# hartikainen/mujoco_mpc

Hardware: AMD Instinct MI355X
Metric: candidate rollouts/s (horizon x samples) (higher is better)
Workload: dtype f64

## Files before the change

mujoco_mpc_amd/csrc/core.h:

```cpp
#pragma once
#include "dmath.h"
#include "model.h"
#include "linalg.h"
#include "philox.h"

#ifdef MJPC_EMU
static thread_local double *g_emu_lds = nullptr;
static thread_local int g_emu_r = 0;
typedef const KParams *KP;
DEV const KParams *kp_generic(KP k) { return k; }
DEV double *lds_base() { return g_emu_lds; }
DEV int cand_index() { return g_emu_r; }
DEV int uniform_i(int v) { return v; }
#else
extern __shared__ __align__(16) double g_lds[];
typedef const __attribute__((address_space(4))) KParams *KP;
DEV const KParams *kp_generic(KP k) {
  unsigned long long v = (unsigned long long)k;
  unsigned lo = __builtin_amdgcn_readfirstlane((unsigned)v), hi = __builtin_amdgcn_readfirstlane((unsigned)(v >> 32));
  KP u = (KP)(((unsigned long long)hi << 32) | lo);
  return (const KParams *)u;
}
DEV double *lds_base() { return g_lds; }
DEV int cand_index() { return (int)blockIdx.x; }
// ... 292 lines not shown
  c.nsingle = nsingle;
  make_contact_rows(c, n_nc); PROF(c, 5);
  make_impedance(c, 0, c.nefc, 1); PROF(c, 7);
#endif
  ctx_close(c);
}
#if MJPC_HELPER
DEV_NOINLINE void ph_noncontact(KP Kc, int t) {
  Ctx c; ctx_open(c, Kc, 1);
  int nsingle, n_nc;
#if MJPC_SIDE_COM
  if (c.M->neq_connect) { if (!flag_wait(c.misc + HX_COM, t + 1)) c.warning |= WARN_SYNC; }
#endif
  make_noncontact_rows(c, &nsingle, &n_nc);
  if (LANE == 0) { c.misc[HX_NC_NSINGLE] = nsingle; c.misc[HX_NC_ROWS] = n_nc; }
  flag_set(c.misc + HX_NCROWS, t + 1);
  PROFW(c, 1);
  make_impedance(c, 0, n_nc, 0);
  PROFW(c, 4);
  if (!flag_wait(c.misc + HX_SWEEP, t + 1)) c.warning |= WARN_SYNC;
  subtree_sums(c, 1);
  flag_set(c.misc + HX_SUBSUM, t + 1);
  PROFW(c, 5);
  ctx_close(c);
}
#endif
template <int NVT>
DEV_NOINLINE void ph_smooth(KP Kc, int t) {
  Ctx c; ctx_open(c, Kc, 1);
#if MJPC_HELPER
#if MJPC_SIDE_COM
  kinematics_rest(c);
  com_pos(c);
  flag_set(c.misc + HX_COM, t + 1);
#endif
  velocity_stage<NVT>(c, Kc, t + 1);
#else
  crb_and_factor<NVT>(c); PROF(c, 3);
  velocity_stage<NVT>(c, Kc, 0); PROF(c, 6);
#endif
  ctx_close(c);
}
#if MJPC_HELPER
template <int NVT>
DEV_NOINLINE void ph_inertia(KP Kc, int t) {
  Ctx c; ctx_open(c, Kc, 1);
#if MJPC_SIDE_COM
  if (!flag_wait(c.misc + HX_COM, t + 1)) c.warning |= WARN_SYNC;
#endif
  crb_and_factor<NVT>(c);
  flag_set(c.misc + HX_MFACT, t + 1);
  ctx_close(c);
}
#endif
template <int NVT>
DEV_NOINLINE void ph_solve(KP Kc, int last, int t) {
  Ctx c; ctx_open(c, Kc);
  c.hseq = t * 256;
  solve_constraints<NVT>(c); PROF(c, 8);
#if MJPC_HELPER
  if (NVT > 0) { if (c.M->cone == 1) flag_set(c.misc + HX_JOBW, JOBW(++c.hseq, 0, 0)); }
  else {
    if (LANE == 0) c.misc[HX_UNREAD_KIND] = 0;
    flag_set(c.misc + HX_UNREAD_SEQ, ++c.hseq);
  }
#endif
  if (!last && !(c.warning & (WARN_CONTACTFULL | WARN_CNSTRFULL)) && bad_values(c.qacc, c.M->nv)) c.warning |= WARN_BADQACC;
  ctx_close(c);
}
template <int NVT>
DEV_NOINLINE void ph_noslip(KP Kc, int last) {
  Ctx c; ctx_open(c, Kc);
  if (!(c.warning & (WARN_CONTACTFULL | WARN_CNSTRFULL | WARN_SYNC | WARN_BADQACC))) {
    noslip_pass<NVT>(c);
    if (!last && bad_values(c.qacc, c.M->nv)) c.warning |= WARN_BADQACC;
  }
  ctx_close(c);
}
#if MJPC_HELPER
template <int NVT>
DEV_NOINLINE void ph_solve_helper(KP Kc, int t) {
  Ctx c; ctx_open(c, Kc, 1);
  int k = WAVE_ID() - 1;
  static_for<0, MJPC_NH>([&](auto Kc_) { constexpr int KK = decltype(Kc_)::value; if (k == KK) solver_helper_loop<NVT, KK>(c, t * 256); });
}
#endif

struct CostOut { double cost; int warning; };
DEV_NOINLINE CostOut ph_residual_cost(KP Kc, int t, int last) {
  Ctx c; ctx_open(c, Kc, 1);
  const KParams *K = c.K;
  const DevModel &M = *c.M;
  const DevTask &T = M.task;
  Rows R = out_rows(K);
  if (last) PFOR(k, M.nu) R.actions[t * M.nu + k] = (K->H > 1) ? c.ctrl[k] : 0.0;
  if (t == 0 && cand_index() == 0 && K->frame) {
    int nb = M.nbody, ns = M.nsite;
    double *f = K->frame;
    PFOR(i, 3 * nb) { f[i] = c.xpos[i]; f[12 * nb + 3 * ns + i] = c.subtree_com[i]; f[15 * nb + 3 * ns + i] = c.subtree_linvel[i]; }
    PFOR(i, 9 * nb) f[3 * nb + i] = c.xmat[i];
    PFOR(i, 3 * ns) f[12 * nb + i] = c.site_xpos[i];
  }
  task_residual(c, c.residual); PROF(c, 9); PROFW(c, 9);
  PFOR(i, R.nr) R.residual[t * R.nr + i] = c.residual[i];
  PFOR(i, T.num_trace) {
    int id = MI(task.trace_objid)[i], ty = MI(task.trace_objtype)[i];
    const double *src = ty == 6 ? c.site_xpos + 3 * id : (ty == 5 ? c.geom_xpos + 3 * id : (ty == 1 ? c.xipos + 3 * id : c.xpos + 3 * id));
    d_copy3(R.trace + t * R.ntr + 3 * i, src);
  }
  CostOut o;
  o.cost = cost_value(c, c.residual);
  if (LANE == 0) R.costs[t] = o.cost;
  o.warning = c.warning;
  PROF(c, 10); PROFW(c, 10);
  ctx_close(c);
  return o;
}

template <int NVT>
DEV void prefactor_body(Ctx &c) {
  const DevModel &M = *c.M;
  {
    int nv = M.nv, nvp = M.nvp;
    double h = M.timestep;
    PFOR(e, nv * nvp) { int i = e / nvp, j = e - i * nvp; c.qL[e] = c.qM[e] + ((i == j) ? h * MD(dof_damping)[i] : 0.0); }
    if (M.nidrv) {
      SYNC();
      if (LANE == 0)
        for (int k = 0; k < M.nidrv; k++) {
          int i = MI(idrv_e)[3 * k], j = MI(idrv_e)[3 * k + 1], a = MI(idrv_e)[3 * k + 2];
          if (a >= 0 && MI(actuator_forcelimited)[a]) {
            double f = c.actuator_force[a];
            if (f <= MD(actuator_forcerange)[2 * a] || f >= MD(actuator_forcerange)[2 * a + 1]) continue;
          }
          double v = h * MD(idrv_c)[k];
          c.qL[i * nvp + j] += v;
          if (i != j) c.qL[j * nvp + i] += v;
        }
      SYNC();
    }
    chol_factor<NVT>(c.qL, c.Linv, c.scr_a, nv, nvp, c.M->tree_ok);
  }
}
template <int NVT>
DEV_NOINLINE void ph_prefactor(KP Kc) {
  Ctx c; ctx_open(c, Kc, 1);
  const DevModel &M = *c.M;
  if (M.any_damping && !M.int_dense && M.noslip_iterations <= 0) prefactor_body<NVT>(c);
  PROFW(c, 11);
  ctx_close(c);
}

DEV void implicit_rne_columns(Ctx &c, double *A, double h) {
  const DevModel &M = *c.M;
  const int nv = M.nv, nvp = M.nvp, nb = M.nbody;
  double *S = lay_ptr(c.K, lds_base(), c.K->L.efc_J);
  int B = M.int_scratch / (18 * nb);
  B = B > NLANE ? NLANE : B;
#define S_(b, k) S[((b) * 18 + (k)) * B + LANE]
  for (int j0 = 0; j0 < nv; j0 += B) {
    const int j = j0 + LANE;
    if (LANE < B && j < nv) {
      for (int pass = 0; pass < 2; pass++) {
        const double sgn = pass ? -1.0 : 1.0;
        for (int b = 1; b < nb; b++) {
          const int p = MIH(body_parentid)[b];
          double cv[6], ca[6];
// ... 286 lines not shown
```

mujoco_mpc_amd/csrc/solver.h:

```cpp
#pragma once
#include "linalg.h"

#ifdef MJPC_EMU
#define LS_RPL 192
#define LS_CPL 64
#else
#define LS_RPL 3
#define LS_CPL 1
#endif

template <int DIMT, bool WRITE = true>
DEV double constraint_update(Ctx &c, int hess, const double *jar) {
  double cost = 0;
  const int nefc = c.nefc, ncon = c.ncon, nv = c.M->nv, nvp = c.M->nvp, stride = c.M->con_stride;
  const int nslot = (nefc + NLANE - 1) / NLANE, ncslot = (ncon + NLANE - 1) / NLANE;
  int rtype[LS_RPL], rdof[LS_RPL];
  double rD[LS_RPL], rx[LS_RPL], rfl[LS_RPL], rR[LS_RPL], rJ[LS_RPL];
  int cdim[LS_CPL], crow[LS_CPL], ctype[LS_CPL];
  double cmu[LS_CPL], cfr[LS_CPL][DIMT], cX[LS_CPL][DIMT], cD[LS_CPL][DIMT];
#pragma unroll
  for (int k = 0; k < LS_RPL; k++) {
    if (k >= nslot) break;
    int i = LANE + NLANE * k, ic = i < nefc ? i : nefc - 1;
    rtype[k] = c.efc_type[ic]; rD[k] = c.efc_D[ic]; rx[k] = jar[ic]; rfl[k] = c.efc_floss[ic]; rR[k] = c.efc_R[ic];
// ... 285 lines not shown
        else {
          i = (int)((sqrtf(8.0f * (float)e + 1.0f) - 1.0f) * 0.5f);
          while ((i + 1) * (i + 2) / 2 <= e) i++;
          while (i * (i + 1) / 2 > e) i--;
          j = e - i * (i + 1) / 2;
        }
      }
      ii[g] = i; jj[g] = j;
    }
    double hp[G], hq[G], hn[G];
#pragma unroll
    for (int g = 0; g < G; g++) { hp[g] = 0; hq[g] = 0; hn[g] = 0; }
    for (int a = 0; a < npos8; a += 8) {
      double x[G][8], y[G][8];
#pragma unroll
      for (int g = 0; g < G; g++)
#pragma unroll
        for (int k = 0; k < 8; k++) { x[g][k] = JH[(a + k) * nvp + ii[g]]; y[g][k] = JH[(a + k) * nvp + jj[g]]; }
#pragma unroll
      for (int g = 0; g < G; g++)
#pragma unroll
        for (int k = 0; k < 8; k += 2) { hp[g] += x[g][k] * y[g][k]; hq[g] += x[g][k + 1] * y[g][k + 1]; }
    }
    for (int a = npos8; a < ntot; a += 4) {
      double x[G][4], y[G][4];
#pragma unroll
      for (int g = 0; g < G; g++)
#pragma unroll
        for (int k = 0; k < 4; k++) { x[g][k] = JH[(a + k) * nvp + ii[g]]; y[g][k] = JH[(a + k) * nvp + jj[g]]; }
#pragma unroll
      for (int g = 0; g < G; g++)
#pragma unroll
        for (int k = 0; k < 4; k++) hn[g] += x[g][k] * y[g][k];
    }
#pragma unroll
    for (int g = 0; g < G; g++) {
      int e = e0 + g * stride, i = ii[g], j = jj[g];
      if (e >= nent) continue;
      double h = hp[g] + hq[g];
      if (j == nv) {
        double gr = c.Ma[i] - c.qfrc_smooth[i] - (c.sgl[i] + c.sgl[2 * nv + i]) - h;
        c.grad[i] = gr;
        c.Mgrad[i] = gr;
      } else {
        h = c.qM[i * nvp + j] + (h - hn[g]);
        if (i == j) h += c.sgl[nv + i] + c.sgl[3 * nv + i];
        c.qH[i * nvp + j] = h;
      }
    }
  }
}

DEV void newton_gradient(Ctx &c, int grad_only) {
  const DevModel &M = *c.M;
  const int nvp = M.nvp;
  PROF(c, 13);
  int npos, nneg;
  newton_lists(c, &npos, &nneg);
  PROF(c, 15);
  newton_fill(c, npos, nneg);
  PROF(c, 19);
  SYNC();
  newton_entries(c, npos, nneg, grad_only);
  if (c.cross) { if (LANE == 0) c.misc[MISC_QH_DENSE] = 1; }
  else {
    PFOR(e, M.nzpair) c.qH[MI(zpair_i)[e] * nvp + MI(zpair_j)[e]] = 0;
    if (LANE == 0) c.misc[MISC_QH_DENSE] = 0;
  }
  SYNC();
  PROF(c, 16);
}

template <int NVT>
DEV double cost_at_smooth(Ctx &c) {
  double *jar = c.efc_pos;
  mat_rows_times<NVT>(c, c.qacc_smooth, c.scr_b, jar);
  PFOR(r, c.nefc) jar[r] -= c.efc_aref[r];
  SYNC();
  double part = c.M->maxdim <= 3 ? constraint_update<3, false>(c, 0, jar) : constraint_update<6, false>(c, 0, jar);
  return 0.0 + wave_sum(part);
}

#if MJPC_HELPER
template <int NVT> DEV void worker_loop(Ctx &c, int W, int last);
template <int NVT> DEV void ls_records_build(Ctx &c);
template <int NVT, int K>
DEV void solver_helper_loop(Ctx &c, int seq) {
  if (K == MJPC_NH - 1 && c.nefc > 0) {
    double cs = cost_at_smooth<NVT>(c);
    if (LANE == 0) c.red[2] = cs;
    const int mute_csm = c.K->fault == 1 && cand_index() == 1 && seq == 2 * 256;
    if (!mute_csm) flag_set(c.misc + HX_CSM, seq / 256 + 1);
  }
  if constexpr (NVT > 0) {
    if (K == 0 && c.nefc > 0) { ls_records_build<NVT>(c); flag_set(c.misc + HX_LSREC, seq / 256 + 1); }
    worker_loop<NVT>(c, K, seq);
  }
}
#endif
template <int NVT>
DEV void newton_direction(Ctx &c) {
  const int nv = NVT > 0 ? NVT : c.M->nv, nvp = NVT > 0 ? NVP_OF(NVT) : c.M->nvp;
  chol_factor_solve<NVT>(c.qH, c.Hinv, c.vtmp, c.Mgrad, nv, nvp, c.M->tree_ok && !c.cross);
  PROF(c, 17);
}
#ifndef MJPC_EMU
template <int NVT>
DEV void newton_direction_sum(Ctx &c, const LDLExtra &ex) {
  chol_factor_solve_reg<NVT>(c.qH, c.Mgrad, NVP_OF(NVT), c.M->tree_ok && !c.cross, &ex);
  PROF(c, 17);
}
#endif

struct LSPoint { double cost, d1, d2; };
template <int DIMT>
struct LSData {
  double lo[LS_RPL], hi[LS_RPL], hD[LS_RPL], F[LS_RPL], X[LS_RPL], V[LS_RPL], DV[LS_RPL], DVV[LS_RPL];
  double U0[LS_CPL][DIMT], UV[LS_CPL][DIMT], E[LS_CPL][DIMT], mu[LS_CPL], Dm[LS_CPL], VV[LS_CPL];
  int on[LS_CPL];
  int nslot, ncslot;
};

template <int DIMT>
DEV void ls_load(Ctx &c, LSData<DIMT> &d) {
  const int nefc = c.nefc, ncon = c.ncon, last = c.nefc - 1;
  d.nslot = (nefc + NLANE - 1) / NLANE; d.ncslot = (ncon + NLANE - 1) / NLANE;
#pragma unroll
  for (int k = 0; k < LS_RPL; k++) {
    d.lo[k] = -1; d.hi[k] = 1; d.hD[k] = 0; d.F[k] = 0; d.X[k] = 0; d.V[k] = 0; d.DV[k] = 0; d.DVV[k] = 0;
    if (k < d.nslot) {
      int r = LANE + NLANE * k, rc = r < nefc ? r : last;
      int type = c.efc_type[rc];
      double D = c.efc_D[rc], v = c.efc_jv[rc], x = c.efc_jar[rc], f = c.efc_floss[rc], Rf = c.efc_R[rc] * f;
      int quad = r < nefc && type != CNSTR_CONTACT_ELLIPTIC;
      int fric = quad && type <= CNSTR_FRICTION_TENDON;
      D = quad ? D : 0.0; v = quad ? v : 0.0;
      d.X[k] = quad ? x : 0.0; d.V[k] = v; d.hD[k] = 0.5 * D; d.DV[k] = D * v; d.DVV[k] = D * v * v;
      d.lo[k] = fric ? -Rf : (quad ? -1e300 : -1.0); d.hi[k] = fric ? Rf : (quad ? 0.0 : 1.0); d.F[k] = fric ? f : 0.0;
    }
  }
#pragma unroll
  for (int q = 0; q < LS_CPL; q++) {
    d.on[q] = 0; d.mu[q] = 0; d.Dm[q] = 0; d.VV[q] = 0;
#pragma unroll
    for (int j = 0; j < DIMT; j++) { d.U0[q][j] = 0; d.UV[q][j] = 0; d.E[q][j] = 0; }
    if (q < d.ncslot) {
      int ci = LANE + NLANE * q, cic = ci < ncon ? ci : ncon - 1;
      int dim = c.con_i[cic * CONI_STRIDE];
      int i = c.con_i[cic * CONI_STRIDE + 3];
      const double *cc = c.contact + cic * c.M->con_stride;
      int type = c.efc_type[i];
      double mu = cc[CON_MU], fr[DIMT], Dj[DIMT], jv[DIMT], jr[DIMT];
#pragma unroll
      for (int j = 0; j < DIMT; j++) {
        int rj = i + j < nefc ? i + j : last;
        fr[j] = j == 0 ? mu : cc[CON_FRICTION + j - 1];
        Dj[j] = c.efc_D[rj]; jv[j] = c.efc_jv[rj]; jr[j] = c.efc_jar[rj];
      }
      int on = ci < ncon && dim > 1 && type == CNSTR_CONTACT_ELLIPTIC;
      d.on[q] = on; d.mu[q] = on ? mu : 0.0;
      d.Dm[q] = on ? Dj[0] * fast_rcp(mu * mu * (1 + mu * mu)) : 0.0;
      double vv = 0;
#pragma unroll
      for (int j = 0; j < DIMT; j++) {
        int use = on && j < dim;
        double uv = jv[j] * fr[j];
        d.U0[q][j] = use ? jr[j] * fr[j] : 0.0; d.UV[q][j] = use ? uv : 0.0;
        d.E[q][j] = use ? Dj[j] * fast_rcp(fr[j] * fr[j]) : 0.0;
        if (j > 0) vv += use ? uv * uv : 0.0;
      }
      d.VV[q] = vv;
    }
  }
}

template <int DIMT>
DEV LSPoint ls_eval(const LSData<DIMT> &d, double q0, double q1, double q2, double a) {
  LSPoint p; p.cost = 0; p.d1 = 0; p.d2 = 0;
#pragma unroll
// ... 165 lines not shown
```

mujoco_mpc_amd/csrc/solver_reg.h:

```cpp
#pragma once
#ifndef MJPC_EMU

template <int NVT> struct HLay {
  static constexpr int G0 = 64 / NVT;
  static constexpr int G = G0 < 1 ? 1 : (G0 > NVT ? NVT : G0);
  static constexpr int CB = (NVT + G - 1) / G;
};
DEV int readlane_i(int v, int lane) { return __builtin_amdgcn_readlane(v, lane); }
#define LSR_STRIDE 7
#define LSC_STRIDE 17
#define LS_ROWREC(c) ((c).efc_JA + 64)
#define LS_CONREC(c) ((c).efc_JA + 64 + (c).M->nefcmax * LSR_STRIDE)

template <int NVT>
DEV void hblock_add_rows(const Ctx &c, double *h, unsigned long long mask, int rbase, double wlane, int hi, int j0) {
  constexpr int nvp = NVP_OF(NVT), CB = HLay<NVT>::CB;
  while (mask) {
    int b0 = (int)__builtin_ctzll(mask); mask &= mask - 1;
    int b1 = b0; double sel1 = 0.0;
    if (mask) { b1 = (int)__builtin_ctzll(mask); mask &= mask - 1; sel1 = 1.0; }
    double w0 = readlane_d(wlane, b0), w1 = readlane_d(wlane, b1) * sel1;
    const double *r0p = c.efc_J + (rbase + b0) * nvp, *r1p = c.efc_J + (rbase + b1) * nvp;
    double x0 = r0p[hi], x1 = r1p[hi];
    double y0[CB], y1[CB];
#pragma unroll
    for (int q = 0; q < CB; q++) { y0[q] = r0p[j0 + q]; y1[q] = r1p[j0 + q]; }
    __builtin_amdgcn_sched_barrier(0);
#ifdef MJPC_LEAN_LDS
    if constexpr (HLay<NVT>::G == 1) {
      double s0 = w0 * x0, s1 = w1 * x1;
#pragma unroll
      for (int q = 0; q < CB; q++) {
        const bool up = j0 + q > hi;
        h[q] = __builtin_fma(up ? w0 * y0[q] : s0, up ? x0 : y0[q], h[q]);
        h[q] = __builtin_fma(up ? w1 * y1[q] : s1, up ? x1 : y1[q], h[q]);
      }
    } else
#endif
    {
      double s0 = w0 * x0, s1 = w1 * x1;
#pragma unroll
      for (int q = 0; q < CB; q++) { h[q] = __builtin_fma(s0, y0[q], h[q]); h[q] = __builtin_fma(s1, y1[q], h[q]); }
    }
  }
}

template <int NVT>
DEV void hblock_init(const Ctx &c, double *hq, int hi, int j0) {
  constexpr int nvp = NVP_OF(NVT), CB = HLay<NVT>::CB;
#pragma unroll
  for (int q = 0; q < CB; q++) hq[q] = c.qM[hi * nvp + j0 + q];
  const int nefc = c.nefc, ns = c.nsingle;
  for (int base = 0; base < nefc; base += NLANE) {
    int r = base + LANE, rc = r < nefc ? r : nefc - 1;
    int st = c.efc_state[rc], type = c.efc_type[rc];
    double D = c.efc_D[rc];
    int flag = r < nefc && r >= ns && st == STATE_QUADRATIC;
    (void)type;
    unsigned long long mask = __builtin_amdgcn_ballot_w64(flag != 0);
    hblock_add_rows<NVT>(c, hq, mask, base, D, hi, j0);
  }
}

template <int NVT>
DEV void newton_grad_reg(Ctx &c, int hi, int hg, bool hact) {
  constexpr int nvp = NVP_OF(NVT), G = HLay<NVT>::G;
  const int ns = c.nsingle, n = c.nefc - ns;
  double part = 0;
  const int trips = (n + G - 1) / G;
  for (int t0 = 0; t0 < trips; t0 += 8) {
    double f[8], j[8];
#pragma unroll
    for (int u = 0; u < 8; u++) {
      int rr = (t0 + u) * G + hg;
      int r = ns + (rr < n ? rr : 0);
      f[u] = c.efc_force[r]; j[u] = c.efc_J[r * nvp + hi];
    }
    __builtin_amdgcn_sched_barrier(0);
#pragma unroll
    for (int u = 0; u < 8; u++) { int rr = (t0 + u) * G + hg; double pr = j[u] * f[u]; part += (rr < n) ? pr : 0.0; }
    __builtin_amdgcn_sched_barrier(0);
  }
  double *sc = c.efc_JA;
  if (hact) sc[hg * NVT + hi] = part;
  SYNC();
  if (LANE < NVT) {
    int i = LANE;
    double jtf = 0;
#pragma unroll
    for (int g = 0; g < G; g++) jtf += sc[g * NVT + i];
    double gr = c.Ma[i] - c.qfrc_smooth[i] - (c.sgl[i] + c.sgl[2 * NVT + i]) - jtf;
    c.grad[i] = gr;
    c.Mgrad[i] = gr;
  }
  SYNC();
}

#define JOBW(seq, np, kind) (((seq) << 4) | ((np) << 2) | (kind))
static_assert(HX_WDONE + MJPC_NH <= HX_WDONE_END, "one done slot per worker");
#define CONE_BASE(c) ((c).efc_JA + 64 + (c).M->nefcmax * LSR_STRIDE + (c).M->nconmax * LSC_STRIDE)
#define CONE_DOFS(c) ((unsigned char *)CONE_BASE(c))
#define CONE_ITEMS(c) ((unsigned short *)(CONE_BASE(c) + ((c).M->nconmax * NVT + 7) / 8))
#define CONE_PARTIAL(c, w) (CONE_BASE(c) + ((c).M->nconmax * NVT + 7) / 8 + ((c).M->nconmax * NVT + 3) / 4 + (w) * (NVT * NVP_OF(NVT)))

template <int NVT, int DIMT>
DEV void cone_rows(const Ctx &c, double *part, int p0, int pstep) {
  constexpr int nvp = NVP_OF(NVT);
  const int nitems = uniform_i(c.misc[HX_NITEMS]), stride = c.M->con_stride;
  const unsigned short *items = CONE_ITEMS(c);
  const double *crec = LS_CONREC(c);
  for (int it0 = p0 * NLANE; it0 < nitems; it0 += pstep * NLANE) {
    const int it = it0 + LANE;
    const bool valid = it < nitems;
    const int item = items[valid ? it : 0];
    const int ci = item & 255, a = item >> 8;
    const int info = ((const int *)(crec + ci * LSC_STRIDE + 14))[0];
    const int r0 = info >> 16, dim = (info >> 8) & 255;
    const unsigned char *dofs = CONE_DOFS(c) + ci * NVT;
    const int i = dofs[a];
    const int st = c.efc_state[r0];
    const double *cf = c.contact + ci * stride + CON_H;
    double P[DIMT], Q[DIMT], T[DIMT], ji[DIMT];
#pragma unroll
    for (int k = 0; k < DIMT; k++) { P[k] = cf[k]; Q[k] = cf[6 + k]; T[k] = cf[12 + k]; }
    const double *Jr = c.efc_J + r0 * nvp;
#pragma unroll
    for (int k = 0; k < DIMT; k++) ji[k] = Jr[(DIMT <= 3 || k < dim ? k : 0) * nvp + i];
    __builtin_amdgcn_sched_barrier(0);
    const bool active = valid && st == STATE_CONE;
#if defined(MJPC_PROFILE) && !defined(MJPC_EMU)
    if (MJPC_PROFILE_WAVE != 0 && WAVE_ID() == MJPC_PROFILE_WAVE) { int na_ = __builtin_popcountll(__builtin_amdgcn_ballot_w64(active)); if (LANE == 0) { c.prof[23] += na_; c.prof[22] += (it0 == p0 * NLANE); } }
#endif
    if constexpr (DIMT > 3) {
#pragma unroll
      for (int k = 3; k < DIMT; k++) { const bool in = k < dim; P[k] = in ? P[k] : 0.0; Q[k] = in ? Q[k] : 0.0; T[k] = in ? T[k] : 0.0; ji[k] = in ? ji[k] : 0.0; }
    }
    double pi = P[0] * ji[0], qi = Q[1] * ji[1];
#pragma unroll
    for (int k = 1; k < DIMT; k++) { pi += P[k] * ji[k]; if (k > 1) qi += Q[k] * ji[k]; }
    double t[DIMT];
    t[0] = P[0] * pi + Q[0] * ji[0];
#pragma unroll
    for (int k = 1; k < DIMT; k++) t[k] = P[k] * pi - Q[k] * qi + (T[k] * T[k]) * ji[k];
    double *prow = part + i * nvp;
    PROFW(c, 16);
    for (int b = 0; __builtin_amdgcn_ballot_w64(active && b <= a) != 0; b += 2) {
      const bool on0 = active && b <= a, on1 = active && b + 1 <= a;
      const int j0 = dofs[on0 ? b : 0], j1 = dofs[on1 ? b + 1 : 0];
      double x0[DIMT], x1[DIMT];
#pragma unroll
      for (int k = 0; k < DIMT; k++) { x0[k] = Jr[(DIMT <= 3 || k < dim ? k : 0) * nvp + j0]; x1[k] = Jr[(DIMT <= 3 || k < dim ? k : 0) * nvp + j1]; }
      __builtin_amdgcn_sched_barrier(0);
      double v0 = t[0] * x0[0], v1 = t[0] * x1[0];
#pragma unroll
      for (int k = 1; k < DIMT; k++) { v0 += t[k] * x0[k]; v1 += t[k] * x1[k]; }
      if (on0) __builtin_amdgcn_ds_atomic_fadd_f64((__attribute__((address_space(3))) double *)(prow + j0), v0);
      if (on1) __builtin_amdgcn_ds_atomic_fadd_f64((__attribute__((address_space(3))) double *)(prow + j1), v1);
    }
  }
}

DEV int jobw_load(const Ctx &c) { return __builtin_amdgcn_readfirstlane(__hip_atomic_load(c.misc + HX_JOBW, __ATOMIC_RELAXED, __HIP_MEMORY_SCOPE_WORKGROUP)); }
DEV int job_post(Ctx &c, int kind, int &side_in) {
  if (c.M->cone != 1) return 0;
  const int seq = ++c.hseq;
  const int np = MJPC_NH + (side_in ? 1 : 0);
  flag_set(c.misc + HX_JOBW, JOBW(seq, np, kind));
  return np;
}
DEV void job_wait(Ctx &c, int np) {
  const int seq = c.hseq;
  for (int k = 0; k < np; k++) if (!flag_wait(c.misc + HX_WDONE + k, seq)) c.warning |= WARN_SYNC;
}
template <int NVT, int DIMT>
DEV void worker_job(Ctx &c, int W, int np, int seq) {
  constexpr int nvp = NVP_OF(NVT);
  PROFW(c, 12);
  double *part = CONE_PARTIAL(c, W);
  PFOR(e, NVT * nvp) part[e] = 0;
  PROFW(c, 15);
  cone_rows<NVT, DIMT>(c, part, W, np);
  PROFW(c, 13);
  flag_set(c.misc + HX_WDONE + W, seq);
  PROFW(c, 14);
}
template <int NVT, int DIMT>
DEV void worker_loop_d(Ctx &c, int W, int last) {
  if (W != 0 && c.nefc > 0 && !flag_wait(c.misc + HX_LSREC, (last >> 8) + 1)) return;
  for (;;) {
    int word = 0, ok = 0;
    for (int n = 0; n < (1 << 21); n++) { word = jobw_load(c); if ((word >> 4) > last) { ok = 1; break; } }
    __builtin_amdgcn_fence(__ATOMIC_ACQUIRE, "workgroup");
    if (!ok) return;
    const int kind = word & 3, np = (word >> 2) & 3;
    if (kind == 0) return;
    last = word >> 4;
    if (W < np) worker_job<NVT, DIMT>(c, W, np, last);
  }
}
template <int NVT>
DEV void worker_loop(Ctx &c, int W, int last) {
  if (c.M->cone != 1) return;
  if (c.M->maxdim <= 3) worker_loop_d<NVT, 3>(c, W, last); else worker_loop_d<NVT, 6>(c, W, last);
}

template <int NVT>
DEV void newton_assemble(Ctx &c, const double *hq, int hi, int hg, int j0, bool hact) {
  constexpr int nvp = NVP_OF(NVT), CB = HLay<NVT>::CB;
  double a[CB];
  const double dg = c.sgl[NVT + hi] + c.sgl[3 * NVT + hi];
#pragma unroll
  for (int q = 0; q < CB; q++) a[q] = hq[q] + ((j0 + q == hi) ? dg : 0.0);
  if (hact) {
#pragma unroll
    for (int q = 0; q < CB; q++) if (j0 + q < NVT) c.qH[hi * nvp + j0 + q] = a[q];
  }
  SYNC();
}
template <int NVT>
DEV void newton_direction_np(Ctx &c, int np) {
  if (np > 0) {
    LDLExtra ex;
    ex.row = nullptr;
    ex.n = np;
#pragma unroll
    for (int w = 0; w < 3; w++) ex.x[w] = CONE_PARTIAL(c, w < np ? w : 0);
    newton_direction_sum<NVT>(c, ex);
  } else newton_direction<NVT>(c);
}

template <int NVT>
DEV void newton_direction_rows(Ctx &c, const double *hq, int hi, bool hact, int np) {
  if constexpr (HLay<NVT>::G != 1) return;
  double row[NVT];
  const double dg = c.sgl[NVT + hi] + c.sgl[3 * NVT + hi];
#pragma unroll
  for (int q = 0; q < NVT; q++) row[q] = hact ? hq[q] + ((q == hi) ? dg : 0.0) : 0.0;
  LDLExtra ex;
  ex.row = row;
  ex.n = np;
#pragma unroll
  for (int w = 0; w < 3; w++) ex.x[w] = CONE_PARTIAL(c, w < np ? w : 0);
  chol_factor_solve_reg<NVT>(c.qH, c.Mgrad, NVP_OF(NVT), c.M->tree_ok && !c.cross, &ex);
  PROF(c, 17);
}

template <int DIMT>
struct LSReg {
  double lo[LS_RPL], hi[LS_RPL], hD[LS_RPL], F[LS_RPL], X[LS_RPL], V[LS_RPL], DV[LS_RPL], DVV[LS_RPL], rJ[LS_RPL];
  int rinfo[LS_RPL];
  double N0[LS_CPL], NV[LS_CPL], t0[LS_CPL], t1[LS_CPL], t2[LS_CPL], c0[LS_CPL], c1[LS_CPL], c2[LS_CPL], mu[LS_CPL], Dm[LS_CPL];
  int on[LS_CPL], cdim[LS_CPL], crow[LS_CPL], cwasq[LS_CPL];
  int nslot, ncslot;
};

template <int NVT>
DEV void ls_records_build(Ctx &c) {
  constexpr int nvp = NVP_OF(NVT);
  const int nefc = c.nefc, ncon = c.ncon, ns = c.nsingle, nfr = c.M->nfric;
  double *rrec = LS_ROWREC(c), *crec = LS_CONREC(c);
  PFOR(r, nefc) {
    int type = c.efc_type[r], dof = c.efc_dof[r];
    double D = c.efc_D[r], f = c.efc_floss[r], Rf = c.efc_R[r] * f;
    int single = r < ns;
    double rj = single ? (r < nfr ? 1.0 : c.efc_J[r * nvp + dof]) : 0.0;
    int quad = type != CNSTR_CONTACT_ELLIPTIC;
    int fric = quad && type <= CNSTR_FRICTION_TENDON;
    double *o = rrec + r * LSR_STRIDE;
    o[0] = fric ? -Rf : (quad ? -1e300 : -1.0); o[1] = fric ? Rf : (quad ? 0.0 : 1.0);
    o[2] = quad ? 0.5 * D : 0.0; o[3] = fric ? f : 0.0; o[4] = rj;
    ((int *)(o + 5))[0] = quad | (fric << 1) | ((quad && single) << 2) | ((single ? dof : 0) << 8);
    o[6] = D;
  }
  int nc_lane = 0;
  PFOR(ci, ncon) {
    int dim = c.con_i[ci * CONI_STRIDE], i = c.con_i[ci * CONI_STRIDE + 3];
    const double *cc = c.contact + ci * c.M->con_stride;
    int on = dim > 1 && c.efc_type[i] == CNSTR_CONTACT_ELLIPTIC;
    double mu = cc[CON_MU];
    double *o = crec + ci * LSC_STRIDE;
    for (int j = 0; j < 6; j++) {
      int use = on && j < dim;
      double fr = j == 0 ? mu : cc[CON_FRICTION + j - 1];
      double Dj = c.efc_D[use ? i + j : i];
      o[j] = use ? Dj * fast_rcp(fr * fr) : 0.0;
      o[6 + j] = use ? fr : 0.0;
// ... 173 lines not shown
      cc[CON_H + 6] = 0;
      cc[CON_H + 12] = -sD * NmT;
#pragma unroll
      for (int j = 1; j < DIMT; j++) if (j < dim) {
        double u = U[j] * iT;
        cc[CON_H + j] = -sD * frj[j] * mu * u;
        cc[CON_H + 6 + j] = sk * frj[j] * u;
        cc[CON_H + 12 + j] = sk * frj[j];
      }
    }
#pragma unroll
    for (int j = 0; j < DIMT; j++) if (j < dim) { c.efc_force[i + j] = F[j]; c.efc_state[i + j] = st; }
    ncone += st == STATE_CONE;
  }
  *ncone_out = __builtin_popcountll(__builtin_amdgcn_ballot_w64(ncone != 0));
#pragma unroll
  for (int k = 0; k < LS_RPL; k++) {
    chg_mask[k] = 0; chg_w[k] = 0;
    if (k >= d.nslot) break;
    int r = LANE + NLANE * k;
    int info = d.rinfo[k];
    const int rc_ = r < nefc ? r : nefc - 1;
    const int st_new = c.efc_state[rc_];
    const double D_ell = LS_ROWREC(c)[rc_ * LSR_STRIDE + 6];
    int quad = info & 1, fric = (info >> 1) & 1, single = (info >> 2) & 1, wasq = (info >> 3) & 1, dof = info >> 8;
    double x = d.X[k] + a * d.V[k];
    if (r < nefc) c.efc_jar[r] = x;
    double lo = d.lo[k], hi = d.hi[k], D = 2 * d.hD[k], f = d.F[k];
    double xc = fmin(fmax(x, lo), hi);
    int inside = x > lo && x < hi;
    int chg = 0;
    cost += d.hD[k] * xc * xc + f * (fabs(x) - fabs(xc));
    if (quad) {
      double force = fric ? (inside ? -D * x : (x <= lo ? f : -f)) : -D * xc;
      c.efc_force[r] = force;
      c.efc_state[r] = inside ? STATE_QUADRATIC : (fric ? (x <= lo ? STATE_LINEARNEG : STATE_LINEARPOS) : STATE_SATISFIED);
      if (single) {
        int kk = fric ? 0 : 2;
        c.sgl[kk * NVT + dof] = d.rJ[k] * force;
        c.sgl[(kk + 1) * NVT + dof] = inside ? D : 0.0;
      } else {
        chg = inside != wasq;
        chg_w[k] = inside ? D : -D;
      }
    } else if (r < nefc) {
      const int nowq = st_new == STATE_QUADRATIC;
      chg = nowq != wasq;
      chg_w[k] = nowq ? D_ell : -D_ell;
    }
    chg_mask[k] = __builtin_amdgcn_ballot_w64(chg != 0);
  }
  return wave_sum(cost);
}

template <int NVT, int DIMT>
DEV void solve_constraints_reg_d(Ctx &c) {
  const DevModel &M = *c.M;
  constexpr int nv = NVT, nvp = NVP_OF(NVT);
  constexpr int G = HLay<NVT>::G, CB = HLay<NVT>::CB;
#ifdef MJPC_LEAN_LDS
  constexpr bool ROWS = G == 1;
#else
  constexpr bool ROWS = false;
#endif
  const int hg_ = LANE / NVT;
  const bool hact = hg_ < G;
  const int hg = hact ? hg_ : 0, hi = hact ? LANE - hg_ * NVT : 0, j0 = hg * CB;
  c.solver_iter = 0;
  PROF(c, 7);
  double gauss, cost, cost_sm;
  double cost_ws = solver_eval<NVT>(c, c.qacc_ws, &gauss);
  if (!flag_wait(c.misc + HX_CSM, c.hseq / 256 + 1)) c.warning |= WARN_SYNC;
  cost_sm = c.red[2];
  if (cost_ws > cost_sm) {
    PFOR(i, nv) c.qacc[i] = c.qacc_smooth[i];
    SYNC();
    cost = solver_eval<NVT>(c, c.qacc, &gauss);
  } else {
    PFOR(i, nv) c.qacc[i] = c.qacc_ws[i];
    SYNC();
    cost = cost_ws;
  }
  PROF(c, 12);
  int np = 0, side_in = 0;
  int ncone = 0;
  if (c.M->cone == 1) {
    const int ci = LANE < c.ncon ? LANE : 0;
    const int dim = c.con_i[ci * CONI_STRIDE], r0c = c.con_i[ci * CONI_STRIDE + 3];
    const int stc = c.efc_state[r0c];
    ncone = __builtin_popcountll(__builtin_amdgcn_ballot_w64(LANE < c.ncon && dim > 1 && stc == STATE_CONE));
  }
  if (ncone) np = job_post(c, 1, side_in);
  double hq[CB];
  hblock_init<NVT>(c, hq, hi, j0);
  PROF(c, 15);
  newton_grad_reg<NVT>(c, hi, hg, hact);
  PROF(c, 9);
  if constexpr (!ROWS) { newton_assemble<NVT>(c, hq, hi, hg, j0, hact); PROF(c, 19); }
  if (np) { job_wait(c, np); PROF(c, 16); }
  if constexpr (!ROWS) newton_direction_np<NVT>(c, np); else newton_direction_rows<NVT>(c, hq, hi, hact, np);
  PFOR(i, nv) c.search[i] = -c.Mgrad[i];
  SYNC();
  const double scale = 1.0 / (M.meaninertia * (nv > 1 ? nv : 1));
  for (int iter = 0; iter < M.iterations; iter++) {
    PROF(c, 13);
    double p_sn = 0, p_q1 = 0, p_q2 = 0, p_gs = 0;
    mat_rows_times<NVT>(c, c.search, c.Mv, c.efc_jv);
    PFOR(i, nv) {
      double si = c.search[i];
      p_sn += si * si; p_q1 += si * (c.Ma[i] - c.qfrc_smooth[i]); p_q2 += 0.5 * si * c.Mv[i]; p_gs += c.grad[i] * si;
    }
    SYNC();
    wave_sum4(p_sn, p_q1, p_q2, p_gs);
    const double snorm = sqrt(p_sn), q1 = p_q1, q2 = p_q2, gs = p_gs;
    PROF(c, 20);
    if (snorm < D_MINVAL || gs >= 0) break;
    const double gtol = M.tolerance * M.ls_tolerance * snorm / scale;
    LSReg<DIMT> d;
    if (iter == 0 && !flag_wait(c.misc + HX_LSREC, c.hseq / 256 + 1)) c.warning |= WARN_SYNC;
    ls_load_reg<NVT, DIMT>(c, d);
    PROF(c, 21);
    double lo = 0, hi_a = -1, a = 1.0;
    double best_a = 0, best_cost = cost, dxold = a, dx = a;
    LSPoint p; p.cost = cost; p.d1 = gs; p.d2 = -gs;
    int moved = 0;
    const double pred_tol = 1e-3 * M.tolerance / scale;
    for (int it = 0; it < M.ls_iterations; it++) {
      p = ls_eval_reg<DIMT>(d, gauss, q1, q2, a);
#if defined(MJPC_PROFILE) && !defined(MJPC_EMU)
      if (LANE == 0) c.prof[23] += 1;
#endif
      int better = p.cost < best_cost;
      best_cost = better ? p.cost : best_cost; best_a = better ? a : best_a;
      int conv = fabs(p.d1) < gtol;
      int neg = p.d1 < 0;
      lo = neg ? a : lo; hi_a = neg ? hi_a : a;
      int pos2 = p.d2 > 0;
      double newton = a - p.d1 * fast_rcp(p.d2);
      double an_e = pos2 ? newton : 2 * a;
      an_e = (an_e > a) ? an_e : 2 * a;
      double nw = pos2 ? newton : lo - 1;
      int ok = (nw > lo) && (nw < hi_a) && (fabs(2 * p.d1) <= fabs(dxold * p.d2));
      double dx_b = ok ? fabs(nw - a) : 0.5 * (hi_a - lo);
      double an_b = ok ? nw : lo + dx_b;
      int bracketed = !(hi_a < 0);
      double an = bracketed ? an_b : an_e;
      dxold = dx; dx = bracketed ? dx_b : an_e - a;
      if (conv || an == a) break;
      const int plain = pos2 && (bracketed ? ok : newton > a);
      if (plain && 0.5 * p.d1 * p.d1 * fast_rcp(p.d2) < pred_tol) { a = an; moved = 1; break; }
      a = an;
    }
    PROF(c, 22);
    const double alpha = moved ? a : best_a;
    PROF(c, 14);
    if (alpha == 0) break;
    unsigned long long chg_mask[LS_RPL]; double chg_w[LS_RPL];
    const double ccost = ls_commit<NVT, DIMT>(c, d, alpha, chg_mask, chg_w, &ncone);
    PFOR(i, nv) { c.qacc[i] += alpha * c.search[i]; c.Ma[i] += alpha * c.Mv[i]; }
    SYNC();
    gauss = gauss + alpha * q1 + alpha * alpha * q2;
    const double oldcost = cost;
    cost = gauss + ccost;
    PROF(c, 12);
    const double improvement = scale * (oldcost - cost);
    const int stop = improvement < M.tolerance || (c.warning & WARN_SYNC) != 0;
    np = (stop || !ncone) ? 0 : job_post(c, 1, side_in);
    if (!stop) {
#pragma unroll
      for (int k = 0; k < LS_RPL; k++) { if (k >= d.nslot) break; hblock_add_rows<NVT>(c, hq, chg_mask[k], NLANE * k, chg_w[k], hi, j0); }
    }
    PROF(c, 15);
    newton_grad_reg<NVT>(c, hi, hg, hact);
    PROF(c, 9);
    c.solver_iter++;
    double pg = 0;
    PFOR(i, nv) pg += c.grad[i] * c.grad[i];
    const double gradient = scale * sqrt(wave_sum(pg));
    const int done = stop || gradient < M.tolerance;
    if constexpr (!ROWS) { if (!done) { newton_assemble<NVT>(c, hq, hi, hg, j0, hact); PROF(c, 19); } }
    if (np) { job_wait(c, np); PROF(c, 16); }
    if (done) break;
    if constexpr (!ROWS) newton_direction_np<NVT>(c, np); else newton_direction_rows<NVT>(c, hq, hi, hact, np);
    PFOR(i, nv) c.search[i] = -c.Mgrad[i];
    SYNC();
  }
  if (LANE == 0) { c.misc[MISC_SUM_ITER] += c.solver_iter; if (c.ncon > c.misc[MISC_MAX_NCON]) c.misc[MISC_MAX_NCON] = c.ncon; if (c.nefc > c.misc[MISC_MAX_NEFC]) c.misc[MISC_MAX_NEFC] = c.nefc; }
  PFOR(i, nv) c.qfrc_constraint[i] = (c.Ma[i] - c.qfrc_smooth[i]) - c.grad[i];
  SYNC();
}

template <int NVT>
DEV void solve_constraints_reg(Ctx &c) {
  if (c.M->maxdim <= 3) solve_constraints_reg_d<NVT, 3>(c); else solve_constraints_reg_d<NVT, 6>(c);
}
#endif
```

Measured before the change: 26310.

## Preload cone Jacobian items into helper-wave registers before job loop

Helper worker waves now preload their first cone item's Jacobian entries, dof indices and row metadata into registers once, before waiting on jobs. Each cone job then uses these cached values for the first pass instead of re-reading LDS. Worker code is moved into a noinline phase that reopens its own context, and the unused side_in path in job_post is dropped. This cuts LDS loads on the critical path of each Newton iteration's cone Hessian assembly, at the cost of more registers per helper wave. The preloaded data is only valid if the item list stays fixed across jobs within a step.

Result: faster. 27940 (median of 6 runs) (+6.2%).

```diff
diff --git a/mujoco_mpc_amd/csrc/core.h b/mujoco_mpc_amd/csrc/core.h
--- a/mujoco_mpc_amd/csrc/core.h
+++ b/mujoco_mpc_amd/csrc/core.h
@@ -398,7 +398,7 @@
 DEV_NOINLINE void ph_solve_helper(KP Kc, int t) {
   Ctx c; ctx_open(c, Kc, 1);
   int k = WAVE_ID() - 1;
-  static_for<0, MJPC_NH>([&](auto Kc_) { constexpr int KK = decltype(Kc_)::value; if (k == KK) solver_helper_loop<NVT, KK>(c, t * 256); });
+  static_for<0, MJPC_NH>([&](auto Kc_) { constexpr int KK = decltype(Kc_)::value; if (k == KK) solver_helper_loop<NVT, KK>(Kc, c, t * 256); });
 }
 #endif
 
diff --git a/mujoco_mpc_amd/csrc/solver.h b/mujoco_mpc_amd/csrc/solver.h
--- a/mujoco_mpc_amd/csrc/solver.h
+++ b/mujoco_mpc_amd/csrc/solver.h
@@ -391,10 +391,10 @@
 }
 
 #if MJPC_HELPER
-template <int NVT> DEV void worker_loop(Ctx &c, int W, int last);
+template <int NVT> DEV void worker_loop(KP Kc, Ctx &c, int W, int last);
 template <int NVT> DEV void ls_records_build(Ctx &c);
 template <int NVT, int K>
-DEV void solver_helper_loop(Ctx &c, int seq) {
+DEV void solver_helper_loop(KP Kc, Ctx &c, int seq) {
   if (K == MJPC_NH - 1 && c.nefc > 0) {
     double cs = cost_at_smooth<NVT>(c);
     if (LANE == 0) c.red[2] = cs;
@@ -403,7 +403,7 @@
   }
   if constexpr (NVT > 0) {
     if (K == 0 && c.nefc > 0) { ls_records_build<NVT>(c); flag_set(c.misc + HX_LSREC, seq / 256 + 1); }
-    worker_loop<NVT>(c, K, seq);
+    worker_loop<NVT>(Kc, c, K, seq);
   }
 }
 #endif
diff --git a/mujoco_mpc_amd/csrc/solver_reg.h b/mujoco_mpc_amd/csrc/solver_reg.h
--- a/mujoco_mpc_amd/csrc/solver_reg.h
+++ b/mujoco_mpc_amd/csrc/solver_reg.h
@@ -103,13 +103,129 @@
 #define CONE_ITEMS(c) ((unsigned short *)(CONE_BASE(c) + ((c).M->nconmax * NVT + 7) / 8))
 #define CONE_PARTIAL(c, w) (CONE_BASE(c) + ((c).M->nconmax * NVT + 7) / 8 + ((c).M->nconmax * NVT + 3) / 4 + (w) * (NVT * NVP_OF(NVT)))
 
-template <int NVT, int DIMT>
-DEV void cone_rows(const Ctx &c, double *part, int p0, int pstep) {
+template <int DIMT>
+DEV void cone_row_t(double *P, double *Q, double *T, double *ji, int dim, double *t) {
+  if constexpr (DIMT > 3) {
+#pragma unroll
+    for (int k = 3; k < DIMT; k++) { const bool in = k < dim; P[k] = in ? P[k] : 0.0; Q[k] = in ? Q[k] : 0.0; T[k] = in ? T[k] : 0.0; ji[k] = in ? ji[k] : 0.0; }
+  }
+  double pi = P[0] * ji[0], qi = Q[1] * ji[1];
+#pragma unroll
+  for (int k = 1; k < DIMT; k++) { pi += P[k] * ji[k]; if (k > 1) qi += Q[k] * ji[k]; }
+  t[0] = P[0] * pi + Q[0] * ji[0];
+#pragma unroll
+  for (int k = 1; k < DIMT; k++) t[k] = P[k] * pi - Q[k] * qi + (T[k] * T[k]) * ji[k];
+}
+template <int DIMT>
+DEV void cone_trip_add(double *prow, const double *t, const double *x0, const double *x1, int j0, int j1, bool on0, bool on1) {
+  double v0 = t[0] * x0[0], v1 = t[0] * x1[0];
+#pragma unroll
+  for (int k = 1; k < DIMT; k++) { v0 += t[k] * x0[k]; v1 += t[k] * x1[k]; }
+  if (on0) __builtin_amdgcn_ds_atomic_fadd_f64((__attribute__((address_space(3))) double *)(prow + j0), v0);
+  if (on1) __builtin_amdgcn_ds_atomic_fadd_f64((__attribute__((address_space(3))) double *)(prow + j1), v1);
+}
+template <int NVT, int DIMT>
+DEV void cone_trips_lds(const unsigned char *dofs, const double *Jr, int dim, double *prow, const double *t, bool active, int a, int b) {
   constexpr int nvp = NVP_OF(NVT);
-  const int nitems = uniform_i(c.misc[HX_NITEMS]), stride = c.M->con_stride;
+  for (; __builtin_amdgcn_ballot_w64(active && b <= a) != 0; b += 2) {
+    const bool on0 = active && b <= a, on1 = active && b + 1 <= a;
+    const int j0 = dofs[on0 ? b : 0], j1 = dofs[on1 ? b + 1 : 0];
+    double x0[DIMT], x1[DIMT];
+#pragma unroll
+    for (int k = 0; k < DIMT; k++) { x0[k] = Jr[(DIMT <= 3 || k < dim ? k : 0) * nvp + j0]; x1[k] = Jr[(DIMT <= 3 || k < dim ? k : 0) * nvp + j1]; }
+    __builtin_amdgcn_sched_barrier(0);
+    cone_trip_add<DIMT>(prow, t, x0, x1, j0, j1, on0, on1);
+  }
+}
+#if defined(MJPC_PROFILE) && !defined(MJPC_EMU)
+#define CONE_PROF_COUNT(c, active, first) do { if (MJPC_PROFILE_WAVE != 0 && WAVE_ID() == MJPC_PROFILE_WAVE) { int na_ = __builtin_popcountll(__builtin_amdgcn_ballot_w64(active)); if (LANE == 0) { (c).prof[23] += na_; (c).prof[22] += (first); } } } while (0)
+#else
+#define CONE_PROF_COUNT(c, active, first) ((void)0)
+#endif
+
+template <int DIMT> struct ConeCap {
+#if defined(MJPC_MIN_BLOCKS) && MJPC_MIN_BLOCKS > 1
+  static constexpr int CAP = DIMT <= 3 ? 10 : 4;
+#else
+  static constexpr int CAP = 10;
+#endif
+};
+template <int NVT, int DIMT>
+struct ConePre {
+  static constexpr int CAP = ConeCap<DIMT>::CAP;
+  int nitems;
+  int valid, a, r0, dim, ci, poff;
+  double ji[DIMT];
+  int j[CAP];
+  double x[CAP][DIMT];
+};
+template <int NVT, int DIMT>
+DEV void cone_preload(const Ctx &c, int W, bool built, ConePre<NVT, DIMT> &p) {
+  constexpr int nvp = NVP_OF(NVT), CAP = ConePre<NVT, DIMT>::CAP;
+  p.nitems = built ? uniform_i(c.misc[HX_NITEMS]) : 0;
+  const int it = W * NLANE + LANE;
+  p.valid = it < p.nitems;
+  p.a = 0; p.r0 = 0; p.dim = 0; p.ci = 0; p.poff = 0;
+#pragma unroll
+  for (int k = 0; k < DIMT; k++) p.ji[k] = 0.0;
+#pragma unroll
+  for (int b = 0; b < CAP; b++) {
+    p.j[b] = 0;
+#pragma unroll
+    for (int k = 0; k < DIMT; k++) p.x[b][k] = 0.0;
+  }
+  if (p.valid) {
+    const int item = CONE_ITEMS(c)[it];
+    p.ci = item & 255; p.a = item >> 8;
+    const int info = ((const int *)(LS_CONREC(c) + p.ci * LSC_STRIDE + 14))[0];
+    p.r0 = info >> 16; p.dim = (info >> 8) & 255;
+    const unsigned char *dofs = CONE_DOFS(c) + p.ci * NVT;
+    const double *Jr = c.efc_J + p.r0 * nvp;
+    const int i = dofs[p.a];
+    p.poff = i * nvp;
+#pragma unroll
+    for (int k = 0; k < DIMT; k++) p.ji[k] = Jr[(DIMT <= 3 || k < p.dim ? k : 0) * nvp + i];
+#pragma unroll
+    for (int b = 0; b < CAP; b++) {
+      const int jb = dofs[b <= p.a ? b : 0];
+      p.j[b] = jb;
+#pragma unroll
+      for (int k = 0; k < DIMT; k++) p.x[b][k] = Jr[(DIMT <= 3 || k < p.dim ? k : 0) * nvp + jb];
+    }
+  }
+}
+
+template <int NVT, int DIMT>
+DEV void cone_rows(const Ctx &c, double *part, int p0, int pstep, const ConePre<NVT, DIMT> &pre) {
+  constexpr int nvp = NVP_OF(NVT), CAP = ConePre<NVT, DIMT>::CAP;
+  const int nitems = pre.nitems, stride = c.M->con_stride;
   const unsigned short *items = CONE_ITEMS(c);
   const double *crec = LS_CONREC(c);
-  for (int it0 = p0 * NLANE; it0 < nitems; it0 += pstep * NLANE) {
+  int it0 = p0 * NLANE;
+  if (it0 < nitems) {
+    const int st = c.efc_state[pre.r0];
+    const double *cf = c.contact + pre.ci * stride + CON_H;
+    double P[DIMT], Q[DIMT], T[DIMT], ji[DIMT], t[DIMT];
+#pragma unroll
+    for (int k = 0; k < DIMT; k++) { P[k] = cf[k]; Q[k] = cf[6 + k]; T[k] = cf[12 + k]; ji[k] = pre.ji[k]; }
+    __builtin_amdgcn_sched_barrier(0);
+    const bool active = pre.valid && st == STATE_CONE;
+    const int a = pre.a;
+    CONE_PROF_COUNT(c, active, 1);
+    cone_row_t<DIMT>(P, Q, T, ji, pre.dim, t);
+    double *prow = part + pre.poff;
+    PROFW(c, 16);
+    int b = 0;
+#pragma unroll
+    for (int u = 0; u < CAP; u += 2) {
+      if (__builtin_amdgcn_ballot_w64(active && u <= a) == 0) break;
+      cone_trip_add<DIMT>(prow, t, pre.x[u], pre.x[u + 1], pre.j[u], pre.j[u + 1], active && u <= a, active && u + 1 <= a);
+      b = u + 2;
+    }
+    cone_trips_lds<NVT, DIMT>(CONE_DOFS(c) + pre.ci * NVT, c.efc_J + pre.r0 * nvp, pre.dim, prow, t, active, a, b);
+    it0 += pstep * NLANE;
+  }
+  for (; it0 < nitems; it0 += pstep * NLANE) {
     const int it = it0 + LANE;
     const bool valid = it < nitems;
     const int item = items[valid ? it : 0];
@@ -128,58 +244,34 @@
     for (int k = 0; k < DIMT; k++) ji[k] = Jr[(DIMT <= 3 || k < dim ? k : 0) * nvp + i];
     __builtin_amdgcn_sched_barrier(0);
     const bool active = valid && st == STATE_CONE;
-#if defined(MJPC_PROFILE) && !defined(MJPC_EMU)
-    if (MJPC_PROFILE_WAVE != 0 && WAVE_ID() == MJPC_PROFILE_WAVE) { int na_ = __builtin_popcountll(__builtin_amdgcn_ballot_w64(active)); if (LANE == 0) { c.prof[23] += na_; c.prof[22] += (it0 == p0 * NLANE); } }
-#endif
-    if constexpr (DIMT > 3) {
-#pragma unroll
-      for (int k = 3; k < DIMT; k++) { const bool in = k < dim; P[k] = in ? P[k] : 0.0; Q[k] = in ? Q[k] : 0.0; T[k] = in ? T[k] : 0.0; ji[k] = in ? ji[k] : 0.0; }
-    }
-    double pi = P[0] * ji[0], qi = Q[1] * ji[1];
-#pragma unroll
-    for (int k = 1; k < DIMT; k++) { pi += P[k] * ji[k]; if (k > 1) qi += Q[k] * ji[k]; }
+    CONE_PROF_COUNT(c, active, 0);
     double t[DIMT];
-    t[0] = P[0] * pi + Q[0] * ji[0];
-#pragma unroll
-    for (int k = 1; k < DIMT; k++) t[k] = P[k] * pi - Q[k] * qi + (T[k] * T[k]) * ji[k];
+    cone_row_t<DIMT>(P, Q, T, ji, dim, t);
     double *prow = part + i * nvp;
     PROFW(c, 16);
-    for (int b = 0; __builtin_amdgcn_ballot_w64(active && b <= a) != 0; b += 2) {
-      const bool on0 = active && b <= a, on1 = active && b + 1 <= a;
-      const int j0 = dofs[on0 ? b : 0], j1 = dofs[on1 ? b + 1 : 0];
-      double x0[DIMT], x1[DIMT];
-#pragma unroll
-      for (int k = 0; k < DIMT; k++) { x0[k] = Jr[(DIMT <= 3 || k < dim ? k : 0) * nvp + j0]; x1[k] = Jr[(DIMT <= 3 || k < dim ? k : 0) * nvp + j1]; }
-      __builtin_amdgcn_sched_barrier(0);
-      double v0 = t[0] * x0[0], v1 = t[0] * x1[0];
-#pragma unroll
-      for (int k = 1; k < DIMT; k++) { v0 += t[k] * x0[k]; v1 += t[k] * x1[k]; }
-      if (on0) __builtin_amdgcn_ds_atomic_fadd_f64((__attribute__((address_space(3))) double *)(prow + j0), v0);
-      if (on1) __builtin_amdgcn_ds_atomic_fadd_f64((__attribute__((address_space(3))) double *)(prow + j1), v1);
-    }
+    cone_trips_lds<NVT, DIMT>(dofs, Jr, dim, prow, t, active, a, 0);
   }
 }
 
 DEV int jobw_load(const Ctx &c) { return __builtin_amdgcn_readfirstlane(__hip_atomic_load(c.misc + HX_JOBW, __ATOMIC_RELAXED, __HIP_MEMORY_SCOPE_WORKGROUP)); }
-DEV int job_post(Ctx &c, int kind, int &side_in) {
+DEV int job_post(Ctx &c, int kind) {
   if (c.M->cone != 1) return 0;
   const int seq = ++c.hseq;
-  const int np = MJPC_NH + (side_in ? 1 : 0);
-  flag_set(c.misc + HX_JOBW, JOBW(seq, np, kind));
-  return np;
+  flag_set(c.misc + HX_JOBW, JOBW(seq, MJPC_NH, kind));
+  return MJPC_NH;
 }
 DEV void job_wait(Ctx &c, int np) {
   const int seq = c.hseq;
   for (int k = 0; k < np; k++) if (!flag_wait(c.misc + HX_WDONE + k, seq)) c.warning |= WARN_SYNC;
 }
 template <int NVT, int DIMT>
-DEV void worker_job(Ctx &c, int W, int np, int seq) {
+DEV void worker_job(Ctx &c, int W, int np, int seq, const ConePre<NVT, DIMT> &pre) {
   constexpr int nvp = NVP_OF(NVT);
   PROFW(c, 12);
   double *part = CONE_PARTIAL(c, W);
   PFOR(e, NVT * nvp) part[e] = 0;
   PROFW(c, 15);
-  cone_rows<NVT, DIMT>(c, part, W, np);
+  cone_rows<NVT, DIMT>(c, part, W, np, pre);
   PROFW(c, 13);
   flag_set(c.misc + HX_WDONE + W, seq);
   PROFW(c, 14);
@@ -187,6 +279,8 @@
 template <int NVT, int DIMT>
 DEV void worker_loop_d(Ctx &c, int W, int last) {
   if (W != 0 && c.nefc > 0 && !flag_wait(c.misc + HX_LSREC, (last >> 8) + 1)) return;
+  ConePre<NVT, DIMT> pre;
+  cone_preload<NVT, DIMT>(c, W, c.nefc > 0, pre);
   for (;;) {
     int word = 0, ok = 0;
     for (int n = 0; n < (1 << 21); n++) { word = jobw_load(c); if ((word >> 4) > last) { ok = 1; break; } }
@@ -195,13 +289,18 @@
     const int kind = word & 3, np = (word >> 2) & 3;
     if (kind == 0) return;
     last = word >> 4;
-    if (W < np) worker_job<NVT, DIMT>(c, W, np, last);
-  }
-}
-template <int NVT>
-DEV void worker_loop(Ctx &c, int W, int last) {
+    if (W < np) worker_job<NVT, DIMT>(c, W, np, last, pre);
+  }
+}
+template <int NVT, int DIMT>
+DEV_NOINLINE void worker_phase(KP Kc, int W, int last) {
+  Ctx c; ctx_open(c, Kc, 1);
+  worker_loop_d<NVT, DIMT>(c, uniform_i(W), uniform_i(last));
+}
+template <int NVT>
+DEV void worker_loop(KP Kc, Ctx &c, int W, int last) {
   if (c.M->cone != 1) return;
-  if (c.M->maxdim <= 3) worker_loop_d<NVT, 3>(c, W, last); else worker_loop_d<NVT, 6>(c, W, last);
+  if (c.M->maxdim <= 3) worker_phase<NVT, 3>(Kc, W, last); else worker_phase<NVT, 6>(Kc, W, last);
 }
 
 template <int NVT>
@@ -541,7 +640,7 @@
     cost = cost_ws;
   }
   PROF(c, 12);
-  int np = 0, side_in = 0;
+  int np = 0;
   int ncone = 0;
   if (c.M->cone == 1) {
     const int ci = LANE < c.ncon ? LANE : 0;
@@ -549,7 +648,7 @@
     const int stc = c.efc_state[r0c];
     ncone = __builtin_popcountll(__builtin_amdgcn_ballot_w64(LANE < c.ncon && dim > 1 && stc == STATE_CONE));
   }
-  if (ncone) np = job_post(c, 1, side_in);
+  if (ncone) np = job_post(c, 1);
   double hq[CB];
   hblock_init<NVT>(c, hq, hi, j0);
   PROF(c, 15);
@@ -624,7 +723,7 @@
     PROF(c, 12);
     const double improvement = scale * (oldcost - cost);
     const int stop = improvement < M.tolerance || (c.warning & WARN_SYNC) != 0;
-    np = (stop || !ncone) ? 0 : job_post(c, 1, side_in);
+    np = (stop || !ncone) ? 0 : job_post(c, 1);
     if (!stop) {
 #pragma unroll
       for (int k = 0; k < LS_RPL; k++) { if (k >= d.nslot) break; hblock_add_rows<NVT>(c, hq, chg_mask[k], NLANE * k, chg_w[k], hi, j0); }
```
